# rostin79s/TFHE-AES

Measured on AMD Instinct MI355X. Metric: AES-128 CTR blocks/sec (FHE), higher is better.
Workload: dtype u64+f64; 1 GPU; configs[2]: 128 CTR blocks per GPU, Server::aes_encrypt 10 rounds (1280 bit-CBS/block), counters pre-incremented client-side; params=PARAM_OPT, blocks_per_gpu=128, total_blocks=128

## Files before the change

### tfhe_aes_amd/csrc/kern_keyswitch.h

```cpp
#pragma once
#include <hip/hip_runtime.h>
#include <stdint.h>
#include "fft_dev.h"

#define KS_CT_TILE 64
#define KS_KSTEP 64

typedef int ks_int4 __attribute__((ext_vector_type(4)));

struct KeyswitchArgs {
    const int8_t *afrag;
    const int8_t *bfrag;
    uint32_t ksteps, coltiles;
    const uint64_t *in;
    uint64_t in_stride;
    int32_t body_index;
    uint32_t body_col;
    uint32_t ncols;
    uint64_t *out;
    uint64_t out_stride, out_z_stride;
    uint64_t m;
};

#define KSL_CT_TILES 8
#define KSL_THREADS (64 * KSL_CT_TILES)
#define KSL_COL_TILES 4

#ifndef FHEAES_KS_DECLS_ONLY
__global__ __launch_bounds__(256) void keybytes_kernel(const uint64_t *key, uint64_t key_z_stride, uint32_t rows, uint32_t ncols,
                                                       uint32_t ksteps, uint32_t coltiles, int8_t *frag)
{
    const uint64_t gid = (uint64_t)blockIdx.x * blockDim.x + threadIdx.x;
    const uint32_t lane = gid & 63;
    const uint64_t t = gid >> 6;
    const uint32_t C = t % coltiles;
    const uint32_t ks = (uint32_t)(t / coltiles);
    const uint32_t z = blockIdx.y;
    if (ks >= ksteps) return;
    const uint32_t col = C * 16 + (lane & 15);
    const uint32_t row0 = ks * KS_KSTEP + (lane >> 4) * 16;
    int8_t b[8][16];
#pragma unroll
    for (int e = 0; e < 16; ++e) {
        uint64_t x = 0;
        if (col < ncols && row0 + e < rows) x = key[(uint64_t)z * key_z_stride + (uint64_t)(row0 + e) * ncols + col];
        uint32_t carry = 0;
#pragma unroll
        for (int j = 0; j < 8; ++j) {
            uint32_t v = (uint32_t)((x >> (8 * j)) & 0xFF) + carry;
            carry = v >= 128 ? 1u : 0u;
            b[j][e] = (int8_t)(v & 0xFF);
        }
    }
    int8_t *o = frag + ((((uint64_t)z * ksteps + ks) * coltiles + C) * 8) * 1024 + (uint64_t)lane * 16;
#pragma unroll
    for (int j = 0; j < 8; ++j) {
        ks_int4 w;
        memcpy(&w, b[j], 16);
        *reinterpret_cast<ks_int4 *>(o + (uint64_t)j * 1024) = w;
    }
}

template <int BASE_LOG, int LEVELS, int PLANES>
__global__ __launch_bounds__(256) void digits_kernel(const uint64_t *in, uint64_t in_stride, uint32_t n_in, uint64_t m,
                                                     uint32_t ksteps, int8_t *frag)
{
    const uint64_t gid = (uint64_t)blockIdx.x * blockDim.x + threadIdx.x;
    const uint32_t lane = gid & 63;
    const uint64_t t = gid >> 6;
    const uint32_t ks = t % ksteps;
    const uint64_t T = t / ksteps;
    const uint64_t ct = T * 16 + (lane & 15);
    const uint32_t q0 = ks * KS_KSTEP + (lane >> 4) * 16;
    int8_t lo[16], hi[16];
#pragma unroll
    for (int e = 0; e < 16; ++e) { lo[e] = 0; hi[e] = 0; }
    if (ct < m) {
        const uint32_t i0 = q0 / LEVELS;
        constexpr int NI = (16 + LEVELS - 1) / LEVELS + 1;
#pragma unroll
        for (int ii = 0; ii < NI; ++ii) {
            const uint32_t i = i0 + ii;
            if (i >= n_in) break;
            int d[LEVELS];
            decompose_all<BASE_LOG, LEVELS>(in[ct * in_stride + i], d);
#pragma unroll
            for (int l = 0; l < LEVELS; ++l) {
                const int e = (int)(i * LEVELS + l) - (int)q0;
                if (e >= 0 && e < 16) {
                    const int dl = ((d[l] + 128) & 255) - 128;
#pragma unroll
                    for (int ee = 0; ee < 16; ++ee) if (ee == e) { lo[ee] = (int8_t)dl; hi[ee] = (int8_t)((d[l] - dl) >> 8); }
                }
            }
        }
    }
    int8_t *o = frag + ((T * ksteps + ks) * PLANES) * 1024 + (uint64_t)lane * 16;
    ks_int4 w;
    memcpy(&w, lo, 16);
    *reinterpret_cast<ks_int4 *>(o) = w;
    if (PLANES == 2) {
        memcpy(&w, hi, 16);
        *reinterpret_cast<ks_int4 *>(o + 1024) = w;
    }
}

template <int PLANES>
__global__ __launch_bounds__(KSL_THREADS, 2) void keyswitch_mfma_lds_kernel(const KeyswitchArgs A)
{
    constexpr int A_FRAGS = KSL_CT_TILES * PLANES;
    constexpr int B_FRAGS = KSL_COL_TILES * 8;
    constexpr int FRAGS = A_FRAGS + B_FRAGS;
    __shared__ __attribute__((aligned(16))) int8_t lds[2 * FRAGS * 1024];
    const int lane = threadIdx.x & 63, wave = threadIdx.x >> 6;
    const int wc = wave & 3, wt = wave >> 2;
    const uint32_t C0 = blockIdx.x * KSL_COL_TILES;
    const uint64_t T0 = (uint64_t)blockIdx.y * KSL_CT_TILES;
    const uint32_t z = blockIdx.z;
    const uint64_t ct_tiles_total = (A.m + 15) / 16;

    ks_int4 acc[4][8];
#pragma unroll
    for (int t = 0; t < 4; ++t)
#pragma unroll
        for (int s = 0; s < 8; ++s) acc[t][s] = (ks_int4){0, 0, 0, 0};

    auto issue = [&](uint32_t ks, int buf) {
        constexpr int WAVES = KSL_THREADS / 64;
#pragma unroll
        for (int i = 0; i < (FRAGS + WAVES - 1) / WAVES; ++i) {
            const int f = wave + WAVES * i;
            if (f < FRAGS) {
                const int8_t *src;
                if (f < A_FRAGS) {
                    uint64_t T = T0 + f / PLANES;
                    if (T >= ct_tiles_total) T = ct_tiles_total - 1;
                    src = A.afrag + ((T * A.ksteps + ks) * PLANES + (f % PLANES)) * 1024;
                } else {
                    const int g = f - A_FRAGS;
                    uint32_t C = C0 + g / 8;
                    if (C >= A.coltiles) C = A.coltiles - 1;
                    src = A.bfrag + ((((uint64_t)z * A.ksteps + ks) * A.coltiles + C) * 8 + (g % 8)) * 1024;
                }
                __builtin_amdgcn_global_load_lds((const __attribute__((address_space(1))) void *)(src + lane * 16),
                                                 (__attribute__((address_space(3))) void *)(lds + ((size_t)buf * FRAGS + f) * 1024), 16, 0, 0);
            }
        }
    };

    issue(0, 0);
    for (uint32_t ks = 0; ks < A.ksteps; ++ks) {
        const int buf = ks & 1;
        asm volatile("s_waitcnt vmcnt(0)" ::: "memory");
        __syncthreads();
        if (ks + 1 < A.ksteps) issue(ks + 1, buf ^ 1);
        const int8_t *base = lds + (size_t)buf * FRAGS * 1024 + lane * 16;
        ks_int4 a[4][PLANES], b[8];
#pragma unroll
        for (int s = 0; s < 8; ++s) b[s] = *reinterpret_cast<const ks_int4 *>(base + (A_FRAGS + wc * 8 + s) * 1024);
#pragma unroll
        for (int t = 0; t < 4; ++t)
#pragma unroll
            for (int pl = 0; pl < PLANES; ++pl) a[t][pl] = *reinterpret_cast<const ks_int4 *>(base + ((wt * 4 + t) * PLANES + pl) * 1024);
#pragma unroll
        for (int s = 0; s < 8; ++s) {
#pragma unroll
            for (int t = 0; t < 4; ++t) acc[t][s] = __builtin_amdgcn_mfma_i32_16x16x64_i8(a[t][0], b[s], acc[t][s], 0, 0, 0);
            if (PLANES == 2 && s >= 1) {
#pragma unroll
                for (int t = 0; t < 4; ++t) acc[t][s] = __builtin_amdgcn_mfma_i32_16x16x64_i8(a[t][1], b[s - 1], acc[t][s], 0, 0, 0);
            }
        }
    }

    const uint32_t C = C0 + wc;
    const uint32_t col = C * 16 + (lane & 15);
    if (C >= A.coltiles || col >= A.ncols) return;
#pragma unroll
    for (int t = 0; t < 4; ++t)
#pragma unroll
        for (int r = 0; r < 4; ++r) {
            const uint64_t ct = (T0 + wt * 4 + t) * 16 + (uint64_t)(lane >> 4) * 4 + r;
            if (ct >= A.m) continue;
            uint64_t v = 0;
#pragma unroll
            for (int s = 0; s < 8; ++s) v += (uint64_t)(int64_t)acc[t][s][r] << (8 * s);
            v = (uint64_t)0 - v;
            if (A.body_index >= 0 && col == A.body_col) v += A.in[ct * A.in_stride + (uint32_t)A.body_index];
            A.out[ct * A.out_stride + (uint64_t)z * A.out_z_stride + col] = v;
        }
}
#endif
```

### tfhe_aes_amd/csrc/ks_launch.h

```cpp
#pragma once
#ifdef FHEAES_SPLIT_KS
#ifndef FHEAES_KS_TU
#define FHEAES_KS_DECLS_ONLY
#endif
#endif
#include "kern_keyswitch.h"

#if defined(FHEAES_SPLIT_KS) && !defined(FHEAES_KS_TU)
#define FHEAES_KS_LAUNCH_DECL
#else
#define FHEAES_KS_LAUNCH_DEFINE
#ifdef FHEAES_SPLIT_KS
#define FHEAES_KS_LAUNCH_LINKAGE
#else
#define FHEAES_KS_LAUNCH_LINKAGE static inline
#endif
#endif

#ifdef FHEAES_KS_LAUNCH_DECL
void ks_launch_digits_k1(dim3 grid, hipStream_t s, const uint64_t *in, uint64_t in_stride, uint32_t n_in, uint64_t m, uint32_t ksteps, int8_t *frag);
void ks_launch_digits_k3(dim3 grid, hipStream_t s, const uint64_t *in, uint64_t in_stride, uint32_t n_in, uint64_t m, uint32_t ksteps, int8_t *frag);
void ks_launch_mfma_lds(int planes, dim3 grid, hipStream_t s, const KeyswitchArgs &a);
void ks_launch_keybytes(dim3 grid, hipStream_t s, const uint64_t *key, uint64_t key_z_stride, uint32_t rows, uint32_t ncols, uint32_t ksteps,
                        uint32_t coltiles, int8_t *frag);
#endif

#ifdef FHEAES_KS_LAUNCH_DEFINE
FHEAES_KS_LAUNCH_LINKAGE void ks_launch_digits_k1(dim3 grid, hipStream_t s, const uint64_t *in, uint64_t in_stride, uint32_t n_in, uint64_t m, uint32_t ksteps, int8_t *frag)
{
    hipLaunchKernelGGL((digits_kernel<2, 6, 1>), grid, dim3(256), 0, s, in, in_stride, n_in, m, ksteps, frag);
}
FHEAES_KS_LAUNCH_LINKAGE void ks_launch_digits_k3(dim3 grid, hipStream_t s, const uint64_t *in, uint64_t in_stride, uint32_t n_in, uint64_t m, uint32_t ksteps, int8_t *frag)
{
    hipLaunchKernelGGL((digits_kernel<12, 3, 2>), grid, dim3(256), 0, s, in, in_stride, n_in, m, ksteps, frag);
}
FHEAES_KS_LAUNCH_LINKAGE void ks_launch_mfma_lds(int planes, dim3 grid, hipStream_t s, const KeyswitchArgs &a)
{
    if (planes == 1) hipLaunchKernelGGL((keyswitch_mfma_lds_kernel<1>), grid, dim3(KSL_THREADS), 0, s, a);
    else hipLaunchKernelGGL((keyswitch_mfma_lds_kernel<2>), grid, dim3(KSL_THREADS), 0, s, a);
}
FHEAES_KS_LAUNCH_LINKAGE void ks_launch_keybytes(dim3 grid, hipStream_t s, const uint64_t *key, uint64_t key_z_stride, uint32_t rows, uint32_t ncols, uint32_t ksteps,
                                          uint32_t coltiles, int8_t *frag)
{
    hipLaunchKernelGGL(keybytes_kernel, grid, dim3(256), 0, s, key, key_z_stride, rows, ncols, ksteps, coltiles, frag);
}
#endif
```

Measured before the change: 60.75 blocks/s.

## Restage keyswitch digit decomposition through LDS with coalesced input loads

The digits kernel is rewritten so each workgroup handles 16 ciphertexts across 12 k-steps. It loads input words with lane-contiguous coalesced reads, decomposes them, scatters the int8 digits into a swizzled LDS image, and then writes the MFMA fragments out with 16-byte stores. The old layout had each lane gather strided words and redundantly decompose overlapping words. The launcher now computes its own grid and ignores the one passed in. The cost is byte-granular LDS scatter writes and a barrier.

```diff
diff --git a/tfhe_aes_amd/csrc/kern_keyswitch.h b/tfhe_aes_amd/csrc/kern_keyswitch.h
--- a/tfhe_aes_amd/csrc/kern_keyswitch.h
+++ b/tfhe_aes_amd/csrc/kern_keyswitch.h
@@ -61,48 +61,64 @@
     }
 }
 
+#define KSD_KSTEPS 12
+#define KSD_THREADS 256
+
+__device__ __forceinline__ uint32_t ksd_image_slot(uint32_t frag, uint32_t rg, uint32_t c, uint32_t planes)
+{
+    const uint32_t group = (frag / planes) * (KS_KSTEP / 16) + rg;
+    return frag * 1024 + rg * 256 + ((c ^ (group & 15)) << 4);
+}
+
 template <int BASE_LOG, int LEVELS, int PLANES>
-__global__ __launch_bounds__(256) void digits_kernel(const uint64_t *in, uint64_t in_stride, uint32_t n_in, uint64_t m,
-                                                     uint32_t ksteps, int8_t *frag)
-{
-    const uint64_t gid = (uint64_t)blockIdx.x * blockDim.x + threadIdx.x;
-    const uint32_t lane = gid & 63;
-    const uint64_t t = gid >> 6;
-    const uint32_t ks = t % ksteps;
-    const uint64_t T = t / ksteps;
-    const uint64_t ct = T * 16 + (lane & 15);
-    const uint32_t q0 = ks * KS_KSTEP + (lane >> 4) * 16;
-    int8_t lo[16], hi[16];
-#pragma unroll
-    for (int e = 0; e < 16; ++e) { lo[e] = 0; hi[e] = 0; }
-    if (ct < m) {
-        const uint32_t i0 = q0 / LEVELS;
-        constexpr int NI = (16 + LEVELS - 1) / LEVELS + 1;
-#pragma unroll
-        for (int ii = 0; ii < NI; ++ii) {
-            const uint32_t i = i0 + ii;
-            if (i >= n_in) break;
+__global__ __launch_bounds__(KSD_THREADS) void digits_kernel(const uint64_t *in, uint64_t in_stride, uint32_t n_in, uint64_t m,
+                                                             uint32_t ksteps, int8_t *frag)
+{
+    static_assert((KSD_KSTEPS * KS_KSTEP) % (64 * LEVELS) == 0, "a workgroup's rows are whole wave loads of whole words");
+    constexpr int WORDS = KSD_KSTEPS * KS_KSTEP / LEVELS;
+    constexpr int LOADS = WORDS / 64;
+    constexpr int CTS = 16 / (KSD_THREADS / 64);
+    __shared__ __attribute__((aligned(16))) int8_t img[KSD_KSTEPS * PLANES * 1024];
+    const uint32_t lane = threadIdx.x & 63, wave = threadIdx.x >> 6;
+    const uint32_t kblocks = (ksteps + KSD_KSTEPS - 1) / KSD_KSTEPS;
+    const uint32_t kb = blockIdx.x % kblocks;
+    const uint64_t T = blockIdx.x / kblocks;
+    const uint32_t i0 = kb * WORDS;
+
+    uint64_t x[CTS][LOADS];
+#pragma unroll
+    for (int c = 0; c < CTS; ++c) {
+        const uint64_t ct = T * 16 + wave * CTS + c;
+#pragma unroll
+        for (int j = 0; j < LOADS; ++j) {
+            const uint32_t i = i0 + j * 64 + lane;
+            x[c][j] = (ct < m && i < n_in) ? in[ct * in_stride + i] : 0;
+        }
+    }
+#pragma unroll
+    for (int j = 0; j < LOADS; ++j) {
+        if (i0 + j * 64 >= n_in) break;
+#pragma unroll
+        for (int c = 0; c < CTS; ++c) {
             int d[LEVELS];
-            decompose_all<BASE_LOG, LEVELS>(in[ct * in_stride + i], d);
+            decompose_all<BASE_LOG, LEVELS>(x[c][j], d);
 #pragma unroll
             for (int l = 0; l < LEVELS; ++l) {
-                const int e = (int)(i * LEVELS + l) - (int)q0;
-                if (e >= 0 && e < 16) {
-                    const int dl = ((d[l] + 128) & 255) - 128;
-#pragma unroll
-                    for (int ee = 0; ee < 16; ++ee) if (ee == e) { lo[ee] = (int8_t)dl; hi[ee] = (int8_t)((d[l] - dl) >> 8); }
-                }
+                const uint32_t q = (j * 64 + lane) * LEVELS + l;
+                const int dl = ((d[l] + 128) & 255) - 128;
+                int8_t *o = img + ksd_image_slot((q / KS_KSTEP) * PLANES, (q % KS_KSTEP) / 16, wave * CTS + c, PLANES) + (q & 15);
+                o[0] = (int8_t)dl;
+                if (PLANES == 2) o[1024] = (int8_t)((d[l] - dl) >> 8);
             }
         }
     }
-    int8_t *o = frag + ((T * ksteps + ks) * PLANES) * 1024 + (uint64_t)lane * 16;
-    ks_int4 w;
-    memcpy(&w, lo, 16);
-    *reinterpret_cast<ks_int4 *>(o) = w;
-    if (PLANES == 2) {
-        memcpy(&w, hi, 16);
-        *reinterpret_cast<ks_int4 *>(o + 1024) = w;
-    }
+    __syncthreads();
+    const uint32_t ks0 = kb * KSD_KSTEPS;
+    const uint32_t slots = (ksteps - ks0 < KSD_KSTEPS ? ksteps - ks0 : KSD_KSTEPS) * PLANES * 64;
+    int8_t *o = frag + ((T * ksteps + ks0) * PLANES) * 1024;
+    for (uint32_t g = threadIdx.x; g < slots; g += KSD_THREADS)
+        *reinterpret_cast<ks_int4 *>(o + (uint64_t)g * 16) =
+            *reinterpret_cast<const ks_int4 *>(img + ksd_image_slot(g >> 6, (g >> 4) & 3, g & 15, PLANES));
 }
 
 template <int PLANES>
diff --git a/tfhe_aes_amd/csrc/ks_launch.h b/tfhe_aes_amd/csrc/ks_launch.h
--- a/tfhe_aes_amd/csrc/ks_launch.h
+++ b/tfhe_aes_amd/csrc/ks_launch.h
@@ -26,13 +26,20 @@
 #endif
 
 #ifdef FHEAES_KS_LAUNCH_DEFINE
+static inline dim3 ks_digits_grid(uint64_t m, uint32_t ksteps)
+{
+    const uint64_t ct_tiles16 = ((m + KS_CT_TILE - 1) / KS_CT_TILE) * (KS_CT_TILE / 16);
+    return dim3((unsigned)(ct_tiles16 * ((ksteps + KSD_KSTEPS - 1) / KSD_KSTEPS)));
+}
 FHEAES_KS_LAUNCH_LINKAGE void ks_launch_digits_k1(dim3 grid, hipStream_t s, const uint64_t *in, uint64_t in_stride, uint32_t n_in, uint64_t m, uint32_t ksteps, int8_t *frag)
 {
-    hipLaunchKernelGGL((digits_kernel<2, 6, 1>), grid, dim3(256), 0, s, in, in_stride, n_in, m, ksteps, frag);
+    (void)grid;
+    hipLaunchKernelGGL((digits_kernel<2, 6, 1>), ks_digits_grid(m, ksteps), dim3(KSD_THREADS), 0, s, in, in_stride, n_in, m, ksteps, frag);
 }
 FHEAES_KS_LAUNCH_LINKAGE void ks_launch_digits_k3(dim3 grid, hipStream_t s, const uint64_t *in, uint64_t in_stride, uint32_t n_in, uint64_t m, uint32_t ksteps, int8_t *frag)
 {
-    hipLaunchKernelGGL((digits_kernel<12, 3, 2>), grid, dim3(256), 0, s, in, in_stride, n_in, m, ksteps, frag);
+    (void)grid;
+    hipLaunchKernelGGL((digits_kernel<12, 3, 2>), ks_digits_grid(m, ksteps), dim3(KSD_THREADS), 0, s, in, in_stride, n_in, m, ksteps, frag);
 }
 FHEAES_KS_LAUNCH_LINKAGE void ks_launch_mfma_lds(int planes, dim3 grid, hipStream_t s, const KeyswitchArgs &a)
 {
```

Result: no change. 60.97 blocks/s, median of 6 (+0.4%).
